# ov2slam/ov2slam

Hardware: AMD Instinct MI355X
Metric: frames/sec tracking + local-BA iters/sec, EuRoC MH_01 stereo 'accurate', 1 GPU vs CPU ref (higher is better)
Workload: dtype u8/int32 fixed point + f32 (LK), f64 (BA)

## Files before the change

### ov2slam_amd/csrc/lk3.hip

```cpp
#include "common.hpp"
#include "xcd_map.hpp"
#include "lk_plan.hpp"
#include <float.h>
#include <math.h>
#include <stdlib.h>
#include <type_traits>

#pragma clang fp contract(off)

struct LK3Params {
    int max_level, max_iter;
    double eps2;
    float min_eig_th;
    int flags;
    float err_th, fb_dist;
    int do_fb;
    int n_max;
};

#define L3_WIN 9
#define L3_RPL 3
#define L3_KPW 20
#define L3_WAVES 1
#define L3_MIN_WAVES_PER_EU 4
#define L3_KPB (L3_KPW * L3_WAVES)
#define L3_IROWS (L3_WIN + 3)
#define L3_JROWS 16
#define L3_NBH_R 3
#define L3_KEEP 8
#define L3_STRIDE 116

struct L3Lv { int w, h, img_pitch, pady; long long img_roi; };

typedef short s16x2 __attribute__((ext_vector_type(2)));
typedef unsigned short u16x2 __attribute__((ext_vector_type(2)));
typedef uint32_t u32x4 __attribute__((ext_vector_type(4)));
typedef uint32_t u32x4_a4 __attribute__((ext_vector_type(4), aligned(4)));
typedef uint32_t u32x3_a1 __attribute__((ext_vector_type(3), aligned(1)));
typedef uint32_t u32x4_a1 __attribute__((ext_vector_type(4), aligned(1)));

__device__ __forceinline__ uint32_t pk_add(uint32_t a, uint32_t b) { return __builtin_bit_cast(uint32_t, __builtin_bit_cast(u16x2, a) + __builtin_bit_cast(u16x2, b)); }
__device__ __forceinline__ uint32_t pk_sub(uint32_t a, uint32_t b) { return __builtin_bit_cast(uint32_t, __builtin_bit_cast(s16x2, a) - __builtin_bit_cast(s16x2, b)); }
__device__ __forceinline__ uint32_t pk_mul(uint32_t a, short c) { return __builtin_bit_cast(uint32_t, __builtin_bit_cast(s16x2, a) * c); }
__device__ __forceinline__ int dot2(uint32_t a, uint32_t b, int c) { return __builtin_amdgcn_sdot2(__builtin_bit_cast(s16x2, a), __builtin_bit_cast(s16x2, b), c, false); }
__device__ __forceinline__ int dot2z(uint32_t a, uint32_t b) { int r; asm("v_dot2_i32_i16 %0, %1, %2, 0" : "=v"(r) : "v"(a), "v"(b)); return r; }
__device__ __forceinline__ int dot2r(uint32_t a, uint32_t b)
{
    int r;
    const int c256 = __builtin_amdgcn_readfirstlane(256);
    asm("v_dot2_i32_i16 %0, %1, %2, %3" : "=v"(r) : "v"(a), "v"(b), "s"(c256));
    return r;
}
__device__ __forceinline__ int dot2h(uint32_t a, uint32_t b)
{
    int r;
    const int c32k = __builtin_amdgcn_readfirstlane(1 << 15);
    asm("v_dot2_i32_i16 %0, %1, %2, %3" : "=v"(r) : "v"(a), "v"(b), "s"(c32k));
    return r;
}
__device__ __forceinline__ int dot2a(uint32_t a, uint32_t b, int c) { int r; asm("v_dot2_i32_i16 %0, %1, %2, %3" : "=v"(r) : "v"(a), "v"(b), "v"(c)); return r; }
template <uint32_t K>
__device__ __forceinline__ uint32_t l3_sel() { uint32_t r; asm("s_mov_b32 %0, %1" : "=s"(r) : "i"(K)); return r; }
__device__ __forceinline__ uint32_t hi16_pair(int s0, int s1) { return __builtin_amdgcn_perm((uint32_t)s1, (uint32_t)s0, l3_sel<0x07060302u>()); }
__device__ __forceinline__ uint32_t shr9_pair(int s0, int s1)
{
    const uint32_t hi8 = __builtin_amdgcn_perm((uint32_t)s1, (uint32_t)s0, l3_sel<0x06050201u>());
    return __builtin_bit_cast(uint32_t, (u16x2)(__builtin_bit_cast(u16x2, hi8) >> (unsigned short)1));
}
__device__ __forceinline__ uint32_t pack_lo16(int lo, int hi) { return __builtin_amdgcn_perm((uint32_t)hi, (uint32_t)lo, 0x05040100u); }
__device__ __forceinline__ uint32_t round9_pair(int s0, int s1)
{
    const uint32_t hi8 = __builtin_amdgcn_perm((uint32_t)s1, (uint32_t)s0, l3_sel<0x06050201u>());
    return __builtin_bit_cast(uint32_t, (u16x2)((__builtin_bit_cast(u16x2, hi8) + (unsigned short)1) >> (unsigned short)1));
}
__device__ __forceinline__ uint32_t odd_pair(uint32_t e_next, uint32_t e) { return __builtin_amdgcn_alignbyte(e_next, e, 2); }
__device__ __forceinline__ uint32_t bytes01(uint32_t w) { return __builtin_amdgcn_perm(0u, w, l3_sel<0x0c010c00u>()); }
__device__ __forceinline__ uint32_t bytes23(uint32_t w) { return __builtin_amdgcn_perm(0u, w, l3_sel<0x0c030c02u>()); }

template <int CTRL>
__device__ __forceinline__ int l3_dpp(int v) { return __builtin_amdgcn_update_dpp(0, v, CTRL, 0xF, 0xF, true); }

__device__ __forceinline__ int l3_sum3(int v, int sub)
{
    int u = v + l3_dpp<0x111>(v);
    u += l3_dpp<0x112>(v);
    const int b1 = l3_dpp<0x101>(u);
    const int b2 = l3_dpp<0x102>(u);
    return sub == 2 ? u : (sub == 1 ? b1 : b2);
}

__device__ __forceinline__ double l3_sum3_exact(int p, int sub)
{
    const int slo = l3_sum3(p & 0xFFFF, sub);
    const int shi = l3_sum3(p >> 16, sub);
    return (double)shi * 65536.0 + (double)slo;
}

__device__ __forceinline__ float l3_sum3_f32(int p, int sub)
{
    const int t = p + l3_dpp<0x111>(p);
    const int q = l3_dpp<0x111>(t);
    const float f = (float)((double)q + (double)p);
    const int fi = __builtin_bit_cast(int, f);
    const int f1 = l3_dpp<0x101>(fi), f2 = l3_dpp<0x102>(fi);
    return __builtin_bit_cast(float, sub == 2 ? fi : (sub == 1 ? f1 : f2));
}

__device__ __forceinline__ int l3_round(float v) { return __float2int_rn(v); }
__device__ __forceinline__ int l3_floor(float v) { return (int)floorf(v); }
__device__ __forceinline__ int l3_m24(int a, int b) { return __mul24(a, b); }
__device__ __forceinline__ int l3_pin(int v) { asm volatile("" : "+v"(v)); return v; }

__device__ __forceinline__ void l3_lds_sync()
{
    __builtin_amdgcn_fence(__ATOMIC_RELEASE, "wavefront");
    __builtin_amdgcn_wave_barrier();
    __builtin_amdgcn_fence(__ATOMIC_ACQUIRE, "wavefront");
}

template <bool CLAMP>
__device__ __forceinline__ void l3_fetch_J_rows(uint32_t *slot, const uint8_t *jroi, const L3Lv &LJ, int xa, uint32_t sh, int jy0, int sub)
{
    sub = l3_pin(sub);
    const uint8_t *p0 = jroi + (long long)(jy0 + sub) * LJ.img_pitch + xa;
    const long long step = 3LL * LJ.img_pitch;
    uint32_t *dst = slot + 48 + 4 * sub;
#pragma unroll
    for (int k = 0; k < 6; k++) {
        if (k < 5 || sub == 0) {
            const uint8_t *p = p0 + k * step;
            if (CLAMP) {
                int y = jy0 + sub + 3 * k;
                y = y < -LJ.pady ? -LJ.pady : (y > LJ.h + LJ.pady - 1 ? LJ.h + LJ.pady - 1 : y);
                p = jroi + (long long)y * LJ.img_pitch + xa;
            }
            *(u32x4 *)(dst + 12 * k) = *(const u32x4_a1 *)(p + sh);
        }
    }
}

__device__ __forceinline__ void l3_fetch_J(uint32_t *slot, const uint8_t *jroi, const L3Lv &LJ, int jx0, int jy0, int sub)
{
    const int xa = jx0 & ~3;
    const uint32_t sh = (uint32_t)(jx0 - xa);
    const bool outside = jy0 < -LJ.pady || jy0 + L3_JROWS - 1 > LJ.h + LJ.pady - 1;
    if (__builtin_amdgcn_ballot_w64(outside) == 0) l3_fetch_J_rows<false>(slot, jroi, LJ, xa, sh, jy0, sub);
    else l3_fetch_J_rows<true>(slot, jroi, LJ, xa, sh, jy0, sub);
}

struct L3Tmpl { uint32_t X[L3_RPL][5], Y[L3_RPL][5]; int cIX, cIY; };

struct L3State {
    float nx, ny;
    int status;
    float err;
    int iters, visits;
};
struct L3Slot { int ax0, ay0, bx0, by0; };

__device__ __forceinline__ void l3_level(const uint8_t *__restrict__ itemI, const L3Lv &LI,
                                         const uint8_t *__restrict__ itemJ, const L3Lv &LJ,
                                         const LK3Params &prm, int level, bool scale_from_input, bool reuse,
                                         float px0, float py0, int sub_, uint32_t *slot, L3State &st, L3Slot &sl)
{
    const int sub = sub_;
    constexpr int WIN = L3_WIN;
    const float halfWin = (float)(WIN - 1) * 0.5f;
    const float FLT_SCALE = 1.f / (float)(1 << 20);
    const float W14 = (float)(1 << 14);
    const float lvl_scale = (float)(1. / (double)(1 << level));

    float prevx = px0 * lvl_scale, prevy = py0 * lvl_scale;
    float nextx, nexty;
    if (scale_from_input) { nextx = st.nx * lvl_scale; nexty = st.ny * lvl_scale; }
    else { nextx = st.nx * 2.f; nexty = st.ny * 2.f; }
    st.nx = nextx; st.ny = nexty;

    prevx -= halfWin; prevy -= halfWin;
    const int ipx = l3_floor(prevx), ipy = l3_floor(prevy);
    if (ipx < -WIN || ipx >= LI.w || ipy < -WIN || ipy >= LI.h) {
        if (level == 0) { st.status = 0; st.err = 0.f; }
        return;
    }
    st.visits++;
    float a = prevx - (float)ipx, b = prevy - (float)ipy;
    int iw00 = l3_round((1.f - a) * (1.f - b) * W14);
    int iw01 = l3_round(a * (1.f - b) * W14);
    int iw10 = l3_round((1.f - a) * b * W14);
    int iw11 = (1 << 14) - iw00 - iw01 - iw10;
    uint32_t W01 = pack_lo16(iw00, iw01), W23 = pack_lo16(iw10, iw11);

    l3_lds_sync();
    const uint8_t *iroi = itemI + LI.img_roi, *jroi = itemJ + LJ.img_roi;
    auto fetch_I = [&](uint32_t *dst, int ixa) {
        const int sub = l3_pin(sub_);
        const bool outside = ipy - 1 < -LI.pady || ipy - 1 + L3_IROWS - 1 > LI.h + LI.pady - 1;
        const bool clamp_rows = __builtin_amdgcn_ballot_w64(outside) != 0;
        const uint8_t *p0 = iroi + (long long)(ipy - 1 + sub) * LI.img_pitch + ixa;
        const long long step = 3LL * LI.img_pitch;
#pragma unroll
        for (int k = 0; k < 4; k++) {
            const uint8_t *p = p0 + k * step;
            if (clamp_rows) {
                int y = ipy - 1 + sub + 3 * k;
                y = y < -LI.pady ? -LI.pady : (y > LI.h + LI.pady - 1 ? LI.h + LI.pady - 1 : y);
                p = iroi + (long long)y * LI.img_pitch + ixa;
            }
            *(u32x4 *)(dst + 4 * sub + 12 * k) = *(const u32x4_a4 *)p;
        }
    };
    const uint32_t *tsrc;
    uint32_t ish;
    int jx0, jy0, jb;
    if (!reuse) {
        const int ixa = (ipx - 1) & ~3;
        ish = (uint32_t)((ipx - 1) - ixa);
        fetch_I(slot, ixa);
        tsrc = slot;
        sl.ax0 = ixa; sl.ay0 = ipy - 1;
        const float sx = nextx - halfWin, sy = nexty - halfWin;
        const int cx0 = l3_floor(fminf(fmaxf(sx, (float)(-WIN)), (float)(LJ.w - 1)));
        const int cy0 = l3_floor(fminf(fmaxf(sy, (float)(-WIN)), (float)(LJ.h - 1)));
        jx0 = cx0 - L3_NBH_R; jy0 = cy0 - L3_NBH_R; jb = 48;
        l3_fetch_J(slot, jroi, LJ, jx0, jy0, sub);
    } else {
        const int sx = ipx - 1 - sl.bx0, sy = ipy - 1 - sl.by0;
        const bool inB = (unsigned)sx <= 3u && (unsigned)sy <= (unsigned)(L3_JROWS - L3_IROWS);
        tsrc = slot + 48 + 4 * sy; ish = (uint32_t)sx;
        if (!inB) {
            const int ixa = (ipx - 1) & ~3;
            ish = (uint32_t)((ipx - 1) - ixa);
            fetch_I(slot + 48, ixa);
            tsrc = slot + 48;
        }
        jx0 = sl.ax0; jy0 = sl.ay0; jb = 0;
    }
    l3_lds_sync();

    L3Tmpl T;
    T.cIX = 0; T.cIY = 0;
    int s11 = 0, s12 = 0, s22 = 0;
    {
        const int r0 = 3 * l3_pin(sub);
        auto load_row = [&](int m, uint32_t (&e)[6]) {
            const u32x3_a1 w = *(const u32x3_a1 *)((const uint8_t *)(tsrc + 4 * (r0 + m)) + ish);
            const uint32_t d0 = w.x, d1 = w.y, d2 = w.z;
            e[0] = bytes01(d0); e[1] = bytes23(d0); e[2] = bytes01(d1); e[3] = bytes23(d1); e[4] = bytes01(d2); e[5] = bytes23(d2);
        };
        const bool border = ipx < 0 || ipx + WIN >= LI.w || ipy + r0 < 0 || ipy + r0 + 3 >= LI.h;
        const bool any_border = __builtin_amdgcn_ballot_w64(border) != 0;
        auto deriv_row = [&](auto border_tag, int d, const uint32_t (&ea)[6], const uint32_t (&eb)[6], const uint32_t (&ec)[6], uint32_t (&dx)[5], uint32_t (&dy)[5]) {
            uint32_t T0[6], T1[6];
#pragma unroll
            for (int i = 0; i < 6; i++) {
                T0[i] = pk_add(pk_mul(pk_add(ea[i], ec[i]), 12), pk_mul(eb[i], 40));
                T1[i] = pk_sub(ec[i], ea[i]);
            }
#pragma unroll
            for (int i = 0; i < 5; i++) {
                dx[i] = pk_sub(T0[i + 1], T0[i]);
                dy[i] = pk_add(pk_mul(pk_add(T1[i], T1[i + 1]), 12), pk_mul(odd_pair(T1[i + 1], T1[i]), 40));
            }
            if constexpr (decltype(border_tag)::value) {
                const int Yd = ipy + r0 + d;
                const bool yin = Yd >= 0 && Yd < LI.h;
                const uint32_t mlo = (uint32_t)l3_pin(0x0000FFFF), mhi = (uint32_t)l3_pin((int)0xFFFF0000u);
#pragma unroll
                for (int i = 0; i < 5; i++) {
                    const int X = ipx + 2 * i;
                    const uint32_t mk = ((yin && X >= 0 && X < LI.w) ? mlo : 0u) | ((yin && X + 1 >= 0 && X + 1 < LI.w) ? mhi : 0u);
                    dx[i] &= mk; dy[i] &= mk;
                }
            }
        };
        auto window_row = [&](int j, const uint32_t (&et)[6], const uint32_t (&eb)[6], const uint32_t (&dxt)[5], const uint32_t (&dyt)[5],
                              const uint32_t (&dxb)[5], const uint32_t (&dyb)[5]) {
            auto taps = [&](int x, int &iv, int &xv, int &yv) {
                const int k = x + 1;
                const uint32_t pt = (k & 1) ? odd_pair(et[(k >> 1) + 1], et[k >> 1]) : et[k >> 1];
                const uint32_t pb = (k & 1) ? odd_pair(eb[(k >> 1) + 1], eb[k >> 1]) : eb[k >> 1];
                iv = dot2(pt, W01, dot2r(pb, W23));
                const uint32_t xt = (x & 1) ? odd_pair(dxt[(x >> 1) + 1], dxt[x >> 1]) : dxt[x >> 1];
                const uint32_t xb = (x & 1) ? odd_pair(dxb[(x >> 1) + 1], dxb[x >> 1]) : dxb[x >> 1];
                const uint32_t yt = (x & 1) ? odd_pair(dyt[(x >> 1) + 1], dyt[x >> 1]) : dyt[x >> 1];
                const uint32_t yb = (x & 1) ? odd_pair(dyb[(x >> 1) + 1], dyb[x >> 1]) : dyb[x >> 1];
                xv = dot2(xt, W01, dot2h(xb, W23));
                yv = dot2(yt, W01, dot2h(yb, W23));
            };
#pragma unroll
            for (int t = 0; t < 5; t++) {
                int i0, x0, y0, i1 = 256, x1 = 0, y1 = 0;
                taps(2 * t, i0, x0, y0);
                if (2 * t + 1 < WIN) taps(2 * t + 1, i1, x1, y1);
                const uint32_t Ipair = shr9_pair(i0, i1);
                T.X[j][t] = hi16_pair(x0, x1);
                T.Y[j][t] = hi16_pair(y0, y1);
                if (j == 0 && t == 0) {
                    s11 = dot2z(T.X[j][t], T.X[j][t]);
                    s12 = dot2z(T.X[j][t], T.Y[j][t]);
                    s22 = dot2z(T.Y[j][t], T.Y[j][t]);
                    T.cIX = dot2z(Ipair, T.X[j][t]);
                    T.cIY = dot2z(Ipair, T.Y[j][t]);
                    continue;
                }
                s11 = dot2(T.X[j][t], T.X[j][t], s11);
                s12 = dot2(T.X[j][t], T.Y[j][t], s12);
                s22 = dot2(T.Y[j][t], T.Y[j][t], s22);
                T.cIX = dot2(Ipair, T.X[j][t], T.cIX);
                T.cIY = dot2(Ipair, T.Y[j][t], T.cIY);
            }
        };
        uint32_t E0[6], E1[6], E2[6], E3[6], DXa[5], DYa[5], DXb[5], DYb[5];
        auto build = [&](auto bt) {
        load_row(0, E0); load_row(1, E1); load_row(2, E2);
        deriv_row(bt, 0, E0, E1, E2, DXa, DYa);
        load_row(3, E3);
        deriv_row(bt, 1, E1, E2, E3, DXb, DYb);
        window_row(0, E1, E2, DXa, DYa, DXb, DYb);
        load_row(4, E0);
        deriv_row(bt, 2, E2, E3, E0, DXa, DYa);
        window_row(1, E2, E3, DXb, DYb, DXa, DYa);
        load_row(5, E1);
        deriv_row(bt, 3, E3, E0, E1, DXb, DYb);
        window_row(2, E3, E0, DXa, DYa, DXb, DYb);
        };
        if (any_border) build(std::true_type());
        else build(std::false_type());
    }
    const float A11 = l3_sum3_f32(s11, sub) * FLT_SCALE;
    const float A12 = l3_sum3_f32(s12, sub) * FLT_SCALE;
    const float A22 = l3_sum3_f32(s22, sub) * FLT_SCALE;
    float D = A11 * A22 - A12 * A12;
    const float minEig = (A22 + A11 - sqrtf((A11 - A22) * (A11 - A22) + 4.f * A12 * A12)) / (float)(2 * WIN * WIN);
    if (prm.flags & OV2_LK_GET_MIN_EIGENVALS) st.err = minEig;
    if (minEig < prm.min_eig_th || D < FLT_EPSILON) {
        if (level == 0) st.status = 0;
        return;
    }
    D = 1.f / D;
    nextx -= halfWin; nexty -= halfWin;
    float pdx = 0.f, pdy = 0.f;
    int it = 0;
    bool active = prm.max_iter > 0;
    while (__builtin_amdgcn_ballot_w64(active) != 0) {
        if (active) {
            const int inx = l3_floor(nextx), iny = l3_floor(nexty);
            const bool oob = inx < -WIN || inx >= LJ.w || iny < -WIN || iny >= LJ.h;
            if (oob) {
                if (level == 0) st.status = 0;
                active = false;
            } else {
                st.iters++;
                a = nextx - (float)inx; b = nexty - (float)iny;
                iw00 = l3_round((1.f - a) * (1.f - b) * W14);
                iw01 = l3_round(a * (1.f - b) * W14);
                iw10 = l3_round((1.f - a) * b * W14);
                iw11 = (1 << 14) - iw00 - iw01 - iw10;
                W01 = pack_lo16(iw00, iw01); W23 = pack_lo16(iw10, iw11);
                int ox = inx - jx0, oy = iny - jy0;
                if ((unsigned)ox > (unsigned)(2 * L3_NBH_R) || (unsigned)oy > (jb ? (unsigned)(2 * L3_NBH_R) : (unsigned)(L3_IROWS - L3_WIN - 1))) {
                    jx0 = inx - L3_NBH_R; jy0 = iny - L3_NBH_R; jb = 48;
                    l3_lds_sync();
                    l3_fetch_J(slot, jroi, LJ, jx0, jy0, sub);
                    l3_lds_sync();
                    ox = L3_NBH_R; oy = L3_NBH_R;
                }
                uint32_t P[4][9];
                const uint8_t *s0 = (const uint8_t *)(slot + jb + 4 * (oy + 3 * sub)) + ox;
#pragma unroll
                for (int m = 0; m < 4; m++) {
                    const u32x3_a1 w = *(const u32x3_a1 *)(s0 + 16 * m);
                    const uint32_t d0 = w.x, d1 = w.y, d2 = w.z;
                    P[m][0] = bytes01(d0); P[m][2] = bytes23(d0); P[m][4] = bytes01(d1); P[m][6] = bytes23(d1); P[m][8] = bytes01(d2);
                    P[m][1] = odd_pair(P[m][2], P[m][0]); P[m][3] = odd_pair(P[m][4], P[m][2]);
                    P[m][5] = odd_pair(P[m][6], P[m][4]); P[m][7] = odd_pair(P[m][8], P[m][6]);
                }
                const int nIX = -T.cIX, nIY = -T.cIY;
                int sb1, sb2;
#pragma unroll
                for (int j = 0; j < L3_RPL; j++) {
                    int v[WIN + 1];
#pragma unroll
                    for (int x = 0; x < WIN; x++) v[x] = dot2(P[j][x], W01, dot2r(P[j + 1][x], W23));
                    v[WIN] = 0;
#pragma unroll
                    for (int t = 0; t < 5; t++) {
                        const uint32_t Jpair = shr9_pair(v[2 * t], v[2 * t + 1]);
                        sb1 = (j == 0 && t == 0) ? dot2a(Jpair, T.X[j][t], nIX) : dot2(Jpair, T.X[j][t], sb1);
                        sb2 = (j == 0 && t == 0) ? dot2a(Jpair, T.Y[j][t], nIY) : dot2(Jpair, T.Y[j][t], sb2);
                    }
                }
                const float b1 = l3_sum3_f32(sb1, sub) * FLT_SCALE;
                const float b2 = l3_sum3_f32(sb2, sub) * FLT_SCALE;
                const float dx = (A12 * b2 - A22 * b1) * D;
                const float dy = (A12 * b1 - A11 * b2) * D;
                nextx += dx; nexty += dy;
                const bool conv_eps = (double)dx * (double)dx + (double)dy * (double)dy <= prm.eps2;
                const bool conv_osc = !conv_eps && it > 0 && fabs((double)(dx + pdx)) < 0.01 && fabs((double)(dy + pdy)) < 0.01;
                st.nx = nextx + halfWin - (conv_osc ? dx * 0.5f : 0.f);
                st.ny = nexty + halfWin - (conv_osc ? dy * 0.5f : 0.f);
                pdx = dx; pdy = dy;
                it++;
                active = !conv_eps && !conv_osc && it < prm.max_iter;
            }
        }
    }
    sl.bx0 = jx0; sl.by0 = jy0;
}

__device__ __forceinline__ void l3_wg_sync()
{
    if (L3_WAVES == 1) l3_lds_sync();
    else __syncthreads();
}

__global__ __launch_bounds__(256) void k_lk_plan(const int *__restrict__ n_per_item, int n_all, int batch, int nbx, int *__restrict__ plan)
{
    __shared__ int s_wave[4];
    const int r = blockIdx.x, lane = threadIdx.x & 63, wave = threadIdx.x >> 6;
    int *list = plan + OV2_LKP_UNITS + (long long)r * ov2_lkp_list_cap(batch, nbx);
    const int entries = ov2_lkp_entries(batch);
    int base = 0;
    for (int j0 = 0; j0 < entries; j0 += 256) {
        const int j = j0 + (int)threadIdx.x;
        ov2_lkp_entry e = {0, 0, 1, 0};
        if (j < entries) {
            const int item = ov2_lkp_item(r, j, batch);
            e = ov2_lkp_entry_of(r, j, batch, nbx, L3_KPB, n_per_item ? n_per_item[item] : n_all);
        }
        int incl = e.count;
        for (int o = 1; o < 64; o <<= 1) {
            const int up = __shfl_up(incl, o);
            if (lane >= o) incl += up;
        }
        if (lane == 63) s_wave[wave] = incl;
        __syncthreads();
        int off = base + incl - e.count;
        for (int w = 0; w < 4; w++) {
            if (w < wave) off += s_wave[w];
            base += s_wave[w];
        }
        for (int t = 0; t < e.count; t++) list[off + t] = ov2_lkp_pack(e.item, e.first + t * e.step, nbx);
        __syncthreads();
    }
    if (threadIdx.x == 0) { plan[OV2_LKP_LEN + r] = base; plan[r * OV2_LKP_CTR_STRIDE] = 0; }
}

__global__ __launch_bounds__(64 * L3_WAVES, L3_MIN_WAVES_PER_EU) void k_fb_klt3(PyrDesc P, PyrDesc C, LK3Params prm, int nbx,
                                                 const float2 *__restrict__ kps, float2 *__restrict__ priors,
                                                 uint8_t *__restrict__ status, float *__restrict__ err_out,
                                                 int *__restrict__ iters_out, const int *__restrict__ n_per_item,
                                                 unsigned long long *__restrict__ stats, int *plan)
{
    __shared__ __attribute__((aligned(16))) uint32_t lds[L3_KPB * L3_STRIDE];
    __shared__ unsigned long long s_stats[2];
    __shared__ int s_pull;
    __shared__ __attribute__((aligned(16))) float keep[L3_KPB * L3_KEEP];
    const int lane = threadIdx.x & 63, wave = threadIdx.x >> 6;
    const int l16 = lane & 15, g = l16 / 3, sub = l16 - 3 * g;
    const int kslot = wave * L3_KPW + (lane >> 4) * 5 + g;
    if (stats) {
        if (threadIdx.x < 2) s_stats[threadIdx.x] = 0;
        __syncthreads();
    }
    int hop = 0;
    for (int round = 0;; round++) {
    int b, bx;
    if (plan) {
        const int cap = ov2_lkp_list_cap(P.batch, nbx);
        int unit = -1;
        while (hop < OV2_LKP_LISTS) {
            const int q = (blockIdx.x + hop) & (OV2_LKP_LISTS - 1);
            int *ctr = plan + q * OV2_LKP_CTR_STRIDE;
            const int len = plan[OV2_LKP_LEN + q];
            if (threadIdx.x == 0) {
                int u = len;
                if (hop == 0 || __hip_atomic_load(ctr, __ATOMIC_RELAXED, __HIP_MEMORY_SCOPE_AGENT) < len) u = (int)atomicAdd((unsigned int *)ctr, 1u);
                s_pull = u;
            }
            l3_wg_sync();
            const int u = __builtin_amdgcn_readfirstlane(s_pull);
            l3_wg_sync();
            if (u < len) { unit = plan[OV2_LKP_UNITS + (long long)q * cap + u]; break; }
            hop++;
        }
        if (unit < 0) break;
        ov2_lkp_unpack(unit, nbx, &b, &bx);
    } else {
        if (round) break;
        ov2_xcd_map(blockIdx.x, nbx, P.batch, &b, &bx);
    }
    const int n = n_per_item ? n_per_item[b] : prm.n_max;
    const int i = bx * L3_KPB + kslot;
    if (l16 < 15 && i < n) {
        uint32_t *slot = lds + kslot * L3_STRIDE;
        float *kk = keep + kslot * L3_KEEP;
        const uint8_t *itemP = P.base + (long long)b * P.item_stride;
        const uint8_t *itemC = C.base + (long long)b * C.item_stride;
        L3State st;
        {
            const long long gi = (long long)b * prm.n_max + i;
            const float2 kp = kps[gi];
            const float2 pr = priors[gi];
            st.nx = (prm.flags & OV2_LK_USE_INITIAL_FLOW) ? pr.x : kp.x;
            st.ny = (prm.flags & OV2_LK_USE_INITIAL_FLOW) ? pr.y : kp.y;
            if (sub == 0) { kk[0] = kp.x; kk[1] = kp.y; }
        }
        st.status = 1; st.err = 0.f; st.iters = 0; st.visits = 0;
        L3Slot sl = {0, 0, 0, 0};
        float fx = 0.f, fy = 0.f;
        const int nsteps = prm.max_level + 1 + (prm.do_fb ? 1 : 0);
        for (int step = 0; step < nsteps; step++) {
            const bool bwd = step > prm.max_level;
            l3_lds_sync();
            if (bwd) {
                fx = st.nx; fy = st.ny;
                int ok = st.status;
                if (ok && st.err > prm.err_th) ok = 0;
                const float W0 = (float)l3_pin(C.lv[0].w), H0 = (float)l3_pin(C.lv[0].h);
                if (ok && !(1.f <= fx && fx < W0 - 1.f && 1.f <= fy && fy < H0 - 1.f)) ok = 0;
                if (sub == 0) {
                    kk[2] = fx; kk[3] = fy; kk[4] = st.err;
                    ((int *)kk)[5] = st.iters; ((int *)kk)[6] = st.visits; ((int *)kk)[7] = ok;
                }
                if (!ok) break;
                st.nx = kk[0]; st.ny = kk[1]; st.status = 1; st.err = 0.f; st.iters = 0; st.visits = 0;
            }
            const int level = bwd ? 0 : prm.max_level - step;
            const bool top = bwd || step == 0;
            const uint8_t *itemI = bwd ? itemC : itemP, *itemJ = bwd ? itemP : itemC;
            L3Lv LI, LJ;
            {
                const PyrLevelDesc &a = P.lv[level], &c = C.lv[level];
                LI.w = bwd ? c.w : a.w; LI.h = bwd ? c.h : a.h; LI.img_pitch = bwd ? c.img_pitch : a.img_pitch;
                LI.pady = bwd ? c.pady : a.pady; LI.img_roi = bwd ? c.img_roi : a.img_roi;
                LJ.w = bwd ? a.w : c.w; LJ.h = bwd ? a.h : c.h; LJ.img_pitch = bwd ? a.img_pitch : c.img_pitch;
                LJ.pady = bwd ? a.pady : c.pady; LJ.img_roi = bwd ? a.img_roi : c.img_roi;
            }
            l3_level(itemI, LI, itemJ, LJ, prm, level, top, bwd, bwd ? fx : kk[0], bwd ? fy : kk[1], sub, slot, st, sl);
        }
        l3_lds_sync();
        if (sub == 0) {
            float ofx, ofy, err_fwd;
            int ok, acc_iters, acc_visits;
            if (prm.do_fb) {
                ofx = kk[2]; ofy = kk[3]; err_fwd = kk[4];
                acc_iters = ((const int *)kk)[5]; acc_visits = ((const int *)kk)[6]; ok = ((const int *)kk)[7];
                if (ok) {
                    acc_iters += st.iters; acc_visits += st.visits;
                    if (!st.status) ok = 0;
                    else {
                        const float ddx = kk[0] - st.nx, ddy = kk[1] - st.ny;
                        const double nrm = sqrt((double)ddx * (double)ddx + (double)ddy * (double)ddy);
                        if (nrm > (double)prm.fb_dist) ok = 0;
                    }
                }
            } else {
                ofx = st.nx; ofy = st.ny; ok = st.status; acc_iters = st.iters; acc_visits = st.visits; err_fwd = st.err;
            }
            const int tid = l3_pin((int)threadIdx.x);
            const int kslot_e = (tid >> 6) * L3_KPW + ((tid & 63) >> 4) * 5 + (tid & 15) / 3;
            const long long gi = (long long)b * prm.n_max + bx * L3_KPB + kslot_e;
            priors[gi] = make_float2(ofx, ofy);
            status[gi] = (uint8_t)ok;
            if (err_out) err_out[gi] = err_fwd;
            if (iters_out) iters_out[gi] = acc_iters;
            if (stats) {
                atomicAdd(&s_stats[0], (unsigned long long)acc_iters);
                atomicAdd(&s_stats[1], (unsigned long long)acc_visits);
            }
        }
    }
    l3_wg_sync();
    }
    if (stats) {
        __syncthreads();
        if (threadIdx.x < 2 && s_stats[threadIdx.x])
            atomicAdd(&stats[(blockIdx.x & (LK_STAT_SLOTS - 1)) * LK_STAT_STRIDE + threadIdx.x], s_stats[threadIdx.x]);
    }
}

int ov2_launch_fb_klt3(ov2_ctx *ctx, const PyrDesc &P, const PyrDesc &C, int max_level, int max_iter, double eps2,
                       float min_eig_th, int flags, float err_th, float fb_dist, int do_fb, int n_max,
                       const float2 *kps, float2 *priors, uint8_t *status, float *err, int *iters,
                       const int *n_per_item, unsigned long long *stats)
{
    LK3Params prm;
    prm.max_level = max_level; prm.max_iter = max_iter; prm.eps2 = eps2; prm.min_eig_th = min_eig_th; prm.flags = flags;
    prm.err_th = err_th; prm.fb_dist = fb_dist; prm.do_fb = do_fb; prm.n_max = n_max;
    const int nbx = (n_max + L3_KPB - 1) / L3_KPB;
    const long long units = (long long)nbx * P.batch;
    OV2_REQUIRE(units <= 0x7FFFFFFF, OV2_EINVAL, "LK launch has more than 2^31 - 1 keypoint blocks");
    hipStream_t s = ctx->stream;
    int grid = (int)units, *plan = nullptr;
    bool persist = ctx->lk_persist > 0;
    if (persist) grid = ctx->lk_persist;
    else if (ctx->lk_persist < 0) {
        if (!ctx->lk_resident_wgs) {
            int per_cu = 0, cus = 0;
            OV2_HIP_CHECK(hipOccupancyMaxActiveBlocksPerMultiprocessor(&per_cu, k_fb_klt3, 64 * L3_WAVES, 0));
            OV2_HIP_CHECK(hipDeviceGetAttribute(&cus, hipDeviceAttributeMultiprocessorCount, ctx->device));
            OV2_REQUIRE(per_cu > 0 && cus > 0, OV2_EHIP, "k_fb_klt3 does not fit the device");
            ctx->lk_resident_wgs = per_cu * cus;
        }
        persist = units > ctx->lk_resident_wgs;
        if (persist) grid = ctx->lk_resident_wgs;
    }
    if (persist) {
        if (int rc = ctx->reserve_lk_plan((size_t)ov2_lkp_ints(P.batch, nbx))) return rc;
        plan = ctx->lk_plan;
        hipLaunchKernelGGL(k_lk_plan, dim3(OV2_LKP_LISTS), dim3(256), 0, s, n_per_item, n_max, P.batch, nbx, plan);
    }
    hipLaunchKernelGGL(k_fb_klt3, dim3(grid), dim3(64 * L3_WAVES), 0, s, P, C, prm, nbx, kps, priors, status, err, iters, n_per_item, stats, plan);
    return OV2_OK;
}
```

### ov2slam_amd/csrc/lk_plan.hpp

```cpp
#pragma once

#if defined(__HIPCC__)
#define OV2_LKP_HD __host__ __device__ __forceinline__
#else
#define OV2_LKP_HD static inline
#endif

#define OV2_LKP_LISTS 8
#define OV2_LKP_CTR_STRIDE 32
#define OV2_LKP_LEN (OV2_LKP_LISTS * OV2_LKP_CTR_STRIDE)
#define OV2_LKP_UNITS (OV2_LKP_LEN + OV2_LKP_LISTS)

struct ov2_lkp_entry { int item, first, step, count; };

OV2_LKP_HD int ov2_lkp_entries(int batch) { return (batch >> 3) + (batch & 7); }
OV2_LKP_HD int ov2_lkp_list_cap(int batch, int nbx) { return nbx * ((batch >> 3) + 1); }
OV2_LKP_HD long long ov2_lkp_ints(int batch, int nbx) { return OV2_LKP_UNITS + (long long)OV2_LKP_LISTS * ov2_lkp_list_cap(batch, nbx); }
OV2_LKP_HD int ov2_lkp_item(int r, int j, int batch) { const int g = batch >> 3; return j < g ? 8 * j + r : 8 * g + (j - g); }
OV2_LKP_HD int ov2_lkp_blocks(int n, int nbx, int kpb) { const int nb = n > 0 ? (n - 1) / kpb + 1 : 0; return nb < nbx ? nb : nbx; }

OV2_LKP_HD ov2_lkp_entry ov2_lkp_entry_of(int r, int j, int batch, int nbx, int kpb, int n)
{
    const int g = batch >> 3, nb = ov2_lkp_blocks(n, nbx, kpb);
    ov2_lkp_entry e;
    if (j < g) { e.item = 8 * j + r; e.first = 0; e.step = 1; e.count = nb; }
    else {
        const int q = j - g;
        e.item = 8 * g + q;
        e.first = (r - q * nbx) & 7;
        e.step = 8;
        e.count = e.first < nb ? (nb - e.first + 7) >> 3 : 0;
    }
    return e;
}

OV2_LKP_HD int ov2_lkp_pack(int item, int block, int nbx) { return item * nbx + block; }
OV2_LKP_HD void ov2_lkp_unpack(int unit, int nbx, int *item, int *block) { *item = unit / nbx; *block = unit - *item * nbx; }

OV2_LKP_HD int ov2_lkp_fill_list(int r, const int *n, int n_all, int batch, int nbx, int kpb, int *list)
{
    int len = 0;
    for (int j = 0; j < ov2_lkp_entries(batch); j++) {
        const int item = ov2_lkp_item(r, j, batch);
        const ov2_lkp_entry e = ov2_lkp_entry_of(r, j, batch, nbx, kpb, n ? n[item] : n_all);
        for (int t = 0; t < e.count; t++) list[len++] = ov2_lkp_pack(e.item, e.first + t * e.step, nbx);
    }
    return len;
}
```

Baseline: 1.231 million.

## Pack keypoints densely across items in persistent LK work lists

Replaces the per-(item, block) unit lists with dense per-list packing, where each work unit covers a contiguous run of keypoints and may span several batch items. Partially filled tail blocks of different items are merged, which is meant to remove idle lanes in the persistent LK kernel when item keypoint counts are not multiples of the block size. Each slot now stores its own item and index in LDS so that image pointers and output indices are per-lane. The cost is a locate walk over entries per unit, a larger plan buffer and more LDS per slot.

After: 1.217 million. -1.2%, worse.

```diff
diff --git a/ov2slam_amd/csrc/lk3.hip b/ov2slam_amd/csrc/lk3.hip
--- a/ov2slam_amd/csrc/lk3.hip
+++ b/ov2slam_amd/csrc/lk3.hip
@@ -27,7 +27,7 @@
 #define L3_IROWS (L3_WIN + 3)
 #define L3_JROWS 16
 #define L3_NBH_R 3
-#define L3_KEEP 8
+#define L3_KEEP 10
 #define L3_STRIDE 116
 
 struct L3Lv { int w, h, img_pitch, pady; long long img_roi; };
@@ -414,36 +414,41 @@
     else __syncthreads();
 }
 
-__global__ __launch_bounds__(256) void k_lk_plan(const int *__restrict__ n_per_item, int n_all, int batch, int nbx, int *__restrict__ plan)
-{
-    __shared__ int s_wave[4];
+__global__ __launch_bounds__(256) void k_lk_plan(const int *__restrict__ n_per_item, int n_max, int batch, int *__restrict__ plan)
+{
+    __shared__ int s_wave[2][4];
     const int r = blockIdx.x, lane = threadIdx.x & 63, wave = threadIdx.x >> 6;
-    int *list = plan + OV2_LKP_UNITS + (long long)r * ov2_lkp_list_cap(batch, nbx);
-    const int entries = ov2_lkp_entries(batch);
-    int base = 0;
-    for (int j0 = 0; j0 < entries; j0 += 256) {
-        const int j = j0 + (int)threadIdx.x;
-        ov2_lkp_entry e = {0, 0, 1, 0};
-        if (j < entries) {
-            const int item = ov2_lkp_item(r, j, batch);
-            e = ov2_lkp_entry_of(r, j, batch, nbx, L3_KPB, n_per_item ? n_per_item[item] : n_all);
-        }
-        int incl = e.count;
+    ov2_lkd_entry *ent = ov2_lkd_entries(plan, r, batch, n_max, L3_KPB);
+    ov2_lkd_unit *unit = ov2_lkd_units(plan, r, batch, n_max, L3_KPB);
+    const int items = ov2_lkd_items(r, batch);
+    int ebase = 0, kbase = 0;
+    for (int j0 = 0; j0 < items; j0 += 256) {
+        const int j = j0 + (int)threadIdx.x, item = 8 * j + r;
+        const int n = j < items ? ov2_lkd_count(n_per_item ? n_per_item[item] : n_max, n_max) : 0;
+        int ie = n > 0, ik = n;
         for (int o = 1; o < 64; o <<= 1) {
-            const int up = __shfl_up(incl, o);
-            if (lane >= o) incl += up;
-        }
-        if (lane == 63) s_wave[wave] = incl;
+            const int ue = __shfl_up(ie, o), uk = __shfl_up(ik, o);
+            if (lane >= o) { ie += ue; ik += uk; }
+        }
+        if (lane == 63) { s_wave[0][wave] = ie; s_wave[1][wave] = ik; }
         __syncthreads();
-        int off = base + incl - e.count;
+        int e = ebase + ie - (n > 0), pre = kbase + ik - n;
         for (int w = 0; w < 4; w++) {
-            if (w < wave) off += s_wave[w];
-            base += s_wave[w];
-        }
-        for (int t = 0; t < e.count; t++) list[off + t] = ov2_lkp_pack(e.item, e.first + t * e.step, nbx);
+            if (w < wave) { e += s_wave[0][w]; pre += s_wave[1][w]; }
+            ebase += s_wave[0][w]; kbase += s_wave[1][w];
+        }
+        if (n > 0) {
+            ent[e] = {item, n};
+            int first;
+            const int cnt = ov2_lkd_units_from(pre, n, L3_KPB, &first);
+            for (int t = 0; t < cnt; t++) unit[first + t] = ov2_lkd_unit_of(first + t, e, item, n, pre, L3_KPB);
+        }
         __syncthreads();
     }
-    if (threadIdx.x == 0) { plan[OV2_LKP_LEN + r] = base; plan[r * OV2_LKP_CTR_STRIDE] = 0; }
+    if (threadIdx.x == 0) {
+        ent[ebase] = ov2_lkd_sentinel();
+        plan[OV2_LKP_LEN + r] = ov2_lkd_len(kbase, L3_KPB); plan[r * OV2_LKP_CTR_STRIDE] = 0;
+    }
 }
 
 __global__ __launch_bounds__(64 * L3_WAVES, L3_MIN_WAVES_PER_EU) void k_fb_klt3(PyrDesc P, PyrDesc C, LK3Params prm, int nbx,
@@ -465,12 +470,12 @@
     }
     int hop = 0;
     for (int round = 0;; round++) {
-    int b, bx;
+    int b = 0, i = 0;
+    bool mine = false;
     if (plan) {
-        const int cap = ov2_lkp_list_cap(P.batch, nbx);
-        int unit = -1;
+        int q = 0, unit = -1;
         while (hop < OV2_LKP_LISTS) {
-            const int q = (blockIdx.x + hop) & (OV2_LKP_LISTS - 1);
+            q = (blockIdx.x + hop) & (OV2_LKP_LISTS - 1);
             int *ctr = plan + q * OV2_LKP_CTR_STRIDE;
             const int len = plan[OV2_LKP_LEN + q];
             if (threadIdx.x == 0) {
@@ -481,22 +486,21 @@
             l3_wg_sync();
             const int u = __builtin_amdgcn_readfirstlane(s_pull);
             l3_wg_sync();
-            if (u < len) { unit = plan[OV2_LKP_UNITS + (long long)q * cap + u]; break; }
+            if (u < len) { unit = u; break; }
             hop++;
         }
         if (unit < 0) break;
-        ov2_lkp_unpack(unit, nbx, &b, &bx);
+        mine = l16 < 15 && ov2_lkd_locate(ov2_lkd_entries(plan, q, P.batch, prm.n_max, L3_KPB), ov2_lkd_units(plan, q, P.batch, prm.n_max, L3_KPB)[unit], kslot, &b, &i);
     } else {
         if (round) break;
+        int bx;
         ov2_xcd_map(blockIdx.x, nbx, P.batch, &b, &bx);
-    }
-    const int n = n_per_item ? n_per_item[b] : prm.n_max;
-    const int i = bx * L3_KPB + kslot;
-    if (l16 < 15 && i < n) {
+        i = bx * L3_KPB + kslot;
+        mine = i < (n_per_item ? n_per_item[b] : prm.n_max);
+    }
+    if (l16 < 15 && mine) {
         uint32_t *slot = lds + kslot * L3_STRIDE;
         float *kk = keep + kslot * L3_KEEP;
-        const uint8_t *itemP = P.base + (long long)b * P.item_stride;
-        const uint8_t *itemC = C.base + (long long)b * C.item_stride;
         L3State st;
         {
             const long long gi = (long long)b * prm.n_max + i;
@@ -504,7 +508,7 @@
             const float2 pr = priors[gi];
             st.nx = (prm.flags & OV2_LK_USE_INITIAL_FLOW) ? pr.x : kp.x;
             st.ny = (prm.flags & OV2_LK_USE_INITIAL_FLOW) ? pr.y : kp.y;
-            if (sub == 0) { kk[0] = kp.x; kk[1] = kp.y; }
+            if (sub == 0) { kk[0] = kp.x; kk[1] = kp.y; ((int *)kk)[8] = b; ((int *)kk)[9] = i; }
         }
         st.status = 1; st.err = 0.f; st.iters = 0; st.visits = 0;
         L3Slot sl = {0, 0, 0, 0};
@@ -528,6 +532,8 @@
             }
             const int level = bwd ? 0 : prm.max_level - step;
             const bool top = bwd || step == 0;
+            const long long item = ((const int *)kk)[8];
+            const uint8_t *itemP = P.base + item * P.item_stride, *itemC = C.base + item * C.item_stride;
             const uint8_t *itemI = bwd ? itemC : itemP, *itemJ = bwd ? itemP : itemC;
             L3Lv LI, LJ;
             {
@@ -558,9 +564,7 @@
             } else {
                 ofx = st.nx; ofy = st.ny; ok = st.status; acc_iters = st.iters; acc_visits = st.visits; err_fwd = st.err;
             }
-            const int tid = l3_pin((int)threadIdx.x);
-            const int kslot_e = (tid >> 6) * L3_KPW + ((tid & 63) >> 4) * 5 + (tid & 15) / 3;
-            const long long gi = (long long)b * prm.n_max + bx * L3_KPB + kslot_e;
+            const long long gi = (long long)((const int *)kk)[8] * prm.n_max + ((const int *)kk)[9];
             priors[gi] = make_float2(ofx, ofy);
             status[gi] = (uint8_t)ok;
             if (err_out) err_out[gi] = err_fwd;
@@ -607,9 +611,10 @@
         if (persist) grid = ctx->lk_resident_wgs;
     }
     if (persist) {
-        if (int rc = ctx->reserve_lk_plan((size_t)ov2_lkp_ints(P.batch, nbx))) return rc;
+        OV2_REQUIRE((long long)ov2_lkd_entry_cap(P.batch) * n_max <= 0x7FFFFFFF, OV2_EINVAL, "LK launch has more than 2^31 - 1 keypoint slots per list");
+        if (int rc = ctx->reserve_lk_plan((size_t)ov2_lkd_ints(P.batch, n_max, L3_KPB))) return rc;
         plan = ctx->lk_plan;
-        hipLaunchKernelGGL(k_lk_plan, dim3(OV2_LKP_LISTS), dim3(256), 0, s, n_per_item, n_max, P.batch, nbx, plan);
+        hipLaunchKernelGGL(k_lk_plan, dim3(OV2_LKP_LISTS), dim3(256), 0, s, n_per_item, n_max, P.batch, plan);
     }
     hipLaunchKernelGGL(k_fb_klt3, dim3(grid), dim3(64 * L3_WAVES), 0, s, P, C, prm, nbx, kps, priors, status, err, iters, n_per_item, stats, plan);
     return OV2_OK;
diff --git a/ov2slam_amd/csrc/lk_plan.hpp b/ov2slam_amd/csrc/lk_plan.hpp
--- a/ov2slam_amd/csrc/lk_plan.hpp
+++ b/ov2slam_amd/csrc/lk_plan.hpp
@@ -47,3 +47,66 @@
     }
     return len;
 }
+
+#define OV2_LKD_LISTS_AT OV2_LKP_UNITS
+
+struct ov2_lkd_entry { int item, n; };
+struct ov2_lkd_unit { int entry, off, item, rem; };
+
+OV2_LKP_HD int ov2_lkd_items(int r, int batch) { return r < batch ? (batch - r + 7) >> 3 : 0; }
+OV2_LKP_HD int ov2_lkd_entry_cap(int batch) { return ((batch + 7) >> 3) + 1; }
+OV2_LKP_HD int ov2_lkd_entry_ints(int batch) { return (2 * ov2_lkd_entry_cap(batch) + 3) & ~3; }
+OV2_LKP_HD long long ov2_lkd_unit_cap(int batch, int n_max, int kpb) { return ((long long)((batch + 7) >> 3) * n_max + kpb - 1) / kpb; }
+OV2_LKP_HD long long ov2_lkd_list_ints(int batch, int n_max, int kpb) { return ov2_lkd_entry_ints(batch) + 4 * ov2_lkd_unit_cap(batch, n_max, kpb); }
+OV2_LKP_HD long long ov2_lkd_ints(int batch, int n_max, int kpb) { return OV2_LKD_LISTS_AT + OV2_LKP_LISTS * ov2_lkd_list_ints(batch, n_max, kpb); }
+OV2_LKP_HD ov2_lkd_entry *ov2_lkd_entries(int *plan, int r, int batch, int n_max, int kpb)
+{
+    return (ov2_lkd_entry *)(plan + OV2_LKD_LISTS_AT + r * ov2_lkd_list_ints(batch, n_max, kpb));
+}
+OV2_LKP_HD ov2_lkd_unit *ov2_lkd_units(int *plan, int r, int batch, int n_max, int kpb)
+{
+    return (ov2_lkd_unit *)(plan + OV2_LKD_LISTS_AT + r * ov2_lkd_list_ints(batch, n_max, kpb) + ov2_lkd_entry_ints(batch));
+}
+OV2_LKP_HD int ov2_lkd_count(int n, int n_max) { return n < 0 ? 0 : (n < n_max ? n : n_max); }
+OV2_LKP_HD int ov2_lkd_len(int total, int kpb) { return (total + kpb - 1) / kpb; }
+OV2_LKP_HD int ov2_lkd_fill(int total, int u, int kpb) { const int left = total - u * kpb; return left < kpb ? left : kpb; }
+OV2_LKP_HD ov2_lkd_entry ov2_lkd_sentinel() { ov2_lkd_entry s; s.item = -1; s.n = 0x7FFFFFFF; return s; }
+
+OV2_LKP_HD int ov2_lkd_units_from(int pre, int n, int kpb, int *first)
+{
+    *first = ov2_lkd_len(pre, kpb);
+    return ov2_lkd_len(pre + n, kpb) - *first;
+}
+OV2_LKP_HD ov2_lkd_unit ov2_lkd_unit_of(int u, int e, int item, int n, int pre, int kpb)
+{
+    ov2_lkd_unit d;
+    d.entry = e; d.off = u * kpb - pre; d.item = item; d.rem = n - d.off;
+    return d;
+}
+
+OV2_LKP_HD bool ov2_lkd_locate(const ov2_lkd_entry *ent, ov2_lkd_unit d, int k, int *item, int *i)
+{
+    if (k < d.rem) { *item = d.item; *i = d.off + k; return true; }
+    int e = d.entry + 1, pos = k - d.rem;
+    ov2_lkd_entry c = ent[e];
+    while (pos >= c.n) { pos -= c.n; c = ent[++e]; }
+    *item = c.item; *i = pos;
+    return c.item >= 0;
+}
+
+OV2_LKP_HD int ov2_lkd_fill_list(int r, const int *n, int n_all, int batch, int n_max, int kpb, ov2_lkd_entry *ent, ov2_lkd_unit *unit, int *n_ent)
+{
+    int e = 0, total = 0;
+    for (int j = 0; j < ov2_lkd_items(r, batch); j++) {
+        const int item = 8 * j + r, c = ov2_lkd_count(n ? n[item] : n_all, n_max);
+        if (c <= 0) continue;
+        ent[e].item = item; ent[e].n = c;
+        int first;
+        const int cnt = ov2_lkd_units_from(total, c, kpb, &first);
+        for (int t = 0; t < cnt; t++) unit[first + t] = ov2_lkd_unit_of(first + t, e, item, c, total, kpb);
+        e++; total += c;
+    }
+    ent[e] = ov2_lkd_sentinel();
+    *n_ent = e;
+    return total;
+}
```
